# mindspore-lab/mindaudio

Hardware: AMD Instinct MI355X
Metric: utterances/s (16 kHz×10 s) fbanks+Conformer fwd, 1/2/4/8 MI355X (higher is better)
Workload: dtype bf16; 1 GPU; features.fbank (n_fft=512 hop=160 n_mels=80, batch-global top_db) on 64 x (10 s @16 kHz) synthetic waves per GPU -> Conformer-small encoder forward (12 blocks, d=256, 4 heads, ff=2048, conv k=15, eval mode) on the (64, 1000, 80) features; random-init weights; global_batch=64, frames=1000

## Files before the change

mindaudio_amd/csrc/subsample_fused.hip:

```cpp
#include <hip/hip_runtime.h>
#include <stdint.h>
#include <stdlib.h>

#include <type_traits>
#include <utility>

#include "../../include/mindaudio_amd.h"

#include "launch.h"

namespace ma {

typedef __attribute__((ext_vector_type(8))) __bf16 sf_bf16x8;
typedef __attribute__((ext_vector_type(4))) float sf_f32x4;
typedef __attribute__((ext_vector_type(2))) __bf16 sf_bf16x2;
typedef __attribute__((ext_vector_type(2))) float sf_f32x2;
typedef __attribute__((address_space(3))) void sf_lds_void_t;

template <int... Is, class F>
__device__ __forceinline__ void sf_static_for_impl(std::integer_sequence<int, Is...>, F&& f) {
  (f(std::integral_constant<int, Is>{}), ...);
}
template <int N, class F>
__device__ __forceinline__ void sf_static_for(F&& f) {
  sf_static_for_impl(std::make_integer_sequence<int, N>{}, f);
}

constexpr int kSfRows = 128, kSfC = 256, kSfThreads = 512;
constexpr int kSfIdim = 80, kSfF1 = 39, kSfF2 = 19;
constexpr int kSfNhoMax = 8;
constexpr int kSfH1Max = 2 * kSfNhoMax + 1;
constexpr int kSfInMax = 2 * kSfH1Max + 1;
constexpr int kSfPosMax = 672;
constexpr int kSfPitch = 80;
constexpr int kSfChunks = 8, kSfTaps = 9;
constexpr int kSfW2Bytes = kSfC * 9 * kSfC * 2;
constexpr int kSfOffX = 11264;
constexpr int kSfOffPatch = kSfOffX + kSfPosMax * 64;
constexpr int kSfPatchBytes = kSfPosMax * kSfPitch;
constexpr int kSfLds = kSfOffPatch + 2 * kSfPatchBytes;
constexpr int kSfOutPitch = 144;
static_assert(kSfInMax * kSfIdim <= 6 * kSfThreads && kSfPosMax <= 2 * kSfThreads && kSfLds <= 163840, "tile geometry");
static_assert(4 * kSfRows * kSfOutPitch <= kSfOffPatch + kSfPatchBytes, "epilogue staging must not reach patch buffer 1");

struct SubsampleFusedParams {
  const float* x;
  int64_t sb, st, sf;
  const float *mean, *istd;
  const char* packed;
  const float* b1;
  const float* b2;
  uint16_t* out;
  int32_t Ho, tiles_per_utt;
};

__device__ __forceinline__ uint32_t sf_pack_bf16(float lo, float hi) {
  const sf_bf16x2 r = __builtin_convertvector((sf_f32x2){lo, hi}, sf_bf16x2);
  return *reinterpret_cast<const uint32_t*>(&r);
}
__device__ __forceinline__ float sf_head(float x) { return __uint_as_float(sf_pack_bf16(x, 0.0f) << 16); }

template <bool IS_W>
__device__ __forceinline__ void sf_split_row(const float (&v)[9], uint32_t (&d)[16]) {
  float h[9], l[9];
#pragma unroll
  for (int t = 0; t < 9; ++t) {
    h[t] = sf_head(v[t]);
    l[t] = v[t] - h[t];
  }
  float k[32];
#pragma unroll
  for (int t = 0; t < 9; ++t) {
    k[t] = h[t];
    k[9 + t] = IS_W ? l[t] : h[t];
    k[18 + t] = IS_W ? h[t] : l[t];
  }
#pragma unroll
  for (int t = 27; t < 32; ++t) k[t] = 0.0f;
#pragma unroll
  for (int j = 0; j < 16; ++j) d[j] = sf_pack_bf16(k[2 * j], k[2 * j + 1]);
}

__global__ void subsample_fused_pack_kernel(const uint16_t* __restrict__ w2, const float* __restrict__ w1, uint4* __restrict__ out) {
  const int idx = blockIdx.x * blockDim.x + threadIdx.x;
  constexpr int kN2 = 4 * kSfChunks * kSfTaps * 4 * 64;
  if (idx < kN2) {
    const int lane = idx & 63, jt = (idx >> 6) & 3, ft = (idx >> 8) % (kSfChunks * kSfTaps), wv = (idx >> 8) / (kSfChunks * kSfTaps);
    const int cc = ft / kSfTaps, tap = ft - cc * kSfTaps;
    const int n = 64 * wv + 16 * jt + (lane & 15);
    out[idx] = *reinterpret_cast<const uint4*>(w2 + (int64_t)n * (9 * kSfC) + tap * kSfC + 32 * cc + 8 * (lane >> 4));
  } else if (idx < kN2 + 16 * 64) {
    const int j = idx - kN2, lane = j & 63, item = j >> 6;
    const int ch = 16 * item + (lane & 15), g = lane >> 4;
    float v[9];
#pragma unroll
    for (int t = 0; t < 9; ++t) v[t] = w1[ch * 9 + t];
    uint32_t d[16];
    sf_split_row<true>(v, d);
    out[idx] = g == 0 ? make_uint4(d[0], d[1], d[2], d[3]) : g == 1 ? make_uint4(d[4], d[5], d[6], d[7])
             : g == 2 ? make_uint4(d[8], d[9], d[10], d[11]) : make_uint4(d[12], d[13], d[14], d[15]);
  }
}

#ifndef SF_PRIO_C
#define SF_PRIO_C 1
#endif
#ifndef SF_PRIO_P
#define SF_PRIO_P 0
#endif
#ifdef MA_SF_PROF
__device__ unsigned long long g_sf_prof[2 * 3 * 32];
#define SF_STAMP(k) do { asm volatile("s_waitcnt lgkmcnt(0)" ::: "memory"); sf_ts[(k)] = __builtin_amdgcn_s_memtime(); asm volatile("s_waitcnt lgkmcnt(0)" ::: "memory"); } while (0)
#define SF_FLUSH(role)                                                                                        \
  do {                                                                                                        \
    const int slot_ = blockIdx.x == 0 ? 0 : blockIdx.x == 1200 ? 1 : blockIdx.x == 2300 ? 2 : -1;             \
    if (slot_ >= 0 && lane == 0)                                                                              \
      for (int k_ = 0; k_ < 32; ++k_) g_sf_prof[((role) * 3 + slot_) * 32 + k_] = sf_ts[k_];                  \
  } while (0)
#else
#define SF_STAMP(k) do { } while (0)
#define SF_FLUSH(role) do { } while (0)
#endif

__global__ __launch_bounds__(kSfThreads, 2) void subsample_fused_kernel(const SubsampleFusedParams p) {
  extern __shared__ __attribute__((aligned(16))) char smem[];
#ifdef MA_SF_PROF
  unsigned long long sf_ts[32] = {};
#endif
  SF_STAMP(0);
  const int tid = threadIdx.x, lane = tid & 63;
  const int wave = __builtin_amdgcn_readfirstlane(tid >> 6);
  const int b = blockIdx.x / p.tiles_per_utt, ti = blockIdx.x - b * p.tiles_per_utt;
  const int npos = p.Ho * kSfF2;
  const int p0 = ti * kSfRows;
  const int np = min(kSfRows, npos - p0);
  const int ho0 = p0 / kSfF2;
  const int nho = (p0 + np - 1) / kSfF2 - ho0 + 1;
  const int nh1 = 2 * nho + 1, nin = 2 * nh1 + 1;
  const int npatch = nh1 * kSfF1;
  float* rows = reinterpret_cast<float*>(smem);
  char* xim = smem + kSfOffX;
  char* patch = smem + kSfOffPatch;

  {
    const float* xb = p.x + (int64_t)b * p.sb + (int64_t)(4 * ho0) * p.st;
    const bool tfast = p.st <= p.sf;
    const int n = nin * kSfIdim;
    float v[6], mu[6], is[6];
    int dst[6];
#pragma unroll
    for (int j = 0; j < 6; ++j) {
      const int i = min(tid + kSfThreads * j, n - 1);
      const int r = tfast ? i % nin : i / kSfIdim, f = tfast ? i / nin : i % kSfIdim;
      dst[j] = r * kSfIdim + f;
      v[j] = xb[r * p.st + f * p.sf];
      mu[j] = p.mean ? p.mean[f] : 0.0f;
      is[j] = p.mean ? p.istd[f] : 1.0f;
    }
#pragma unroll
    for (int j = 0; j < 6; ++j)
      if (tid + kSfThreads * j < n) rows[dst[j]] = p.mean ? (v[j] - mu[j]) * is[j] : v[j];
  }
  __syncthreads();
  SF_STAMP(1);
#pragma unroll
  for (int j = 0; j < 2; ++j) {
    const int pos = tid + kSfThreads * j;
    if (pos < kSfPosMax) {
      uint32_t d[16];
      if (pos < npatch) {
        const int h = pos / kSfF1, w = pos - h * kSfF1;
        const float* in = rows + (2 * h) * kSfIdim + 2 * w;
        float v[9];
#pragma unroll
        for (int kh = 0; kh < 3; ++kh)
#pragma unroll
          for (int kw = 0; kw < 3; ++kw) v[kh * 3 + kw] = in[kh * kSfIdim + kw];
        sf_split_row<false>(v, d);
      } else {
#pragma unroll
        for (int q = 0; q < 16; ++q) d[q] = 0u;
      }
      uint4* xo = reinterpret_cast<uint4*>(xim + pos * 64);
      xo[0] = make_uint4(d[0], d[1], d[2], d[3]);
      xo[1] = make_uint4(d[4], d[5], d[6], d[7]);
      xo[2] = make_uint4(d[8], d[9], d[10], d[11]);
      xo[3] = make_uint4(d[12], d[13], d[14], d[15]);
    }
  }
  __syncthreads();
  SF_STAMP(2);

  const int ci = lane & 15, gi = lane >> 4;
  auto build_patch = [&](int cc, int pw, int nprod) __attribute__((always_inline)) {
    const uint4* w1f = reinterpret_cast<const uint4*>(p.packed + kSfW2Bytes) + (2 * cc) * 64 + lane;
    const uint4 wa = w1f[0], wb = w1f[64];
    const sf_bf16x8 a0 = *reinterpret_cast<const sf_bf16x8*>(&wa), a1 = *reinterpret_cast<const sf_bf16x8*>(&wb);
    const float4 ba = *reinterpret_cast<const float4*>(p.b1 + 32 * cc + 4 * gi);
    const float4 bb = *reinterpret_cast<const float4*>(p.b1 + 32 * cc + 16 + 4 * gi);
    const sf_f32x4 c0 = {ba.x, ba.y, ba.z, ba.w}, c1 = {bb.x, bb.y, bb.z, bb.w};
    const char* xsrc = xim + ci * 64 + gi * 16;
    char* dst = patch + (cc & 1) * kSfPatchBytes + ci * kSfPitch + gi * 8;
    const int ntile = (npatch + 15) >> 4;
    for (int pt = pw; pt < ntile; pt += nprod) {
      const uint4 xr = *reinterpret_cast<const uint4*>(xsrc + pt * (16 * 64));
      const sf_bf16x8 xf = *reinterpret_cast<const sf_bf16x8*>(&xr);
      const sf_f32x4 d0 = __builtin_amdgcn_mfma_f32_16x16x32_bf16(a0, xf, c0, 0, 0, 0);
      const sf_f32x4 d1 = __builtin_amdgcn_mfma_f32_16x16x32_bf16(a1, xf, c1, 0, 0, 0);
      char* o = dst + pt * (16 * kSfPitch);
      *reinterpret_cast<uint2*>(o) = make_uint2(sf_pack_bf16(fmaxf(d0[0], 0.f), fmaxf(d0[1], 0.f)), sf_pack_bf16(fmaxf(d0[2], 0.f), fmaxf(d0[3], 0.f)));
      *reinterpret_cast<uint2*>(o + 32) = make_uint2(sf_pack_bf16(fmaxf(d1[0], 0.f), fmaxf(d1[1], 0.f)), sf_pack_bf16(fmaxf(d1[2], 0.f), fmaxf(d1[3], 0.f)));
    }
  };
  build_patch(0, wave, 8);
  SF_STAMP(3);

  if (wave >= 4) {
#if SF_PRIO_P
    __builtin_amdgcn_s_setprio(SF_PRIO_P);
#endif
#pragma unroll 1
    for (int k = 0; k + 1 < kSfChunks; ++k) {
      __syncthreads();
      SF_STAMP(4 + 2 * k);
      build_patch(k + 1, wave - 4, 4);
      SF_STAMP(5 + 2 * k);
    }
    __syncthreads();
    SF_STAMP(20);
    if (wave == 4) SF_FLUSH(1);
    return;
  }

#if SF_PRIO_C
  __builtin_amdgcn_s_setprio(SF_PRIO_C);
#endif
  const int c = lane & 15, g = lane >> 4;
  uint32_t a_addr[8];
#pragma unroll
  for (int s = 0; s < 8; ++s) {
    int m = 16 * s + c;
    if (m >= np) m = np - 1;
    const int pos = p0 + m, ho = pos / kSfF2, wo = pos - ho * kSfF2;
    a_addr[s] = (uint32_t)(uintptr_t)(sf_lds_void_t*)(patch + ((2 * (ho - ho0)) * kSfF1 + 2 * wo) * kSfPitch + g * 16);
  }
  const uint32_t voff = lane * 16 + 2048;
  const char* wbase = p.packed + (int64_t)wave * (kSfChunks * kSfTaps) * 4096;
#define SF_LOAD(dst, ft, jt)                                                                                          \
  do {                                                                                                                \
    const char* cb_ = wbase + (int64_t)((ft) < kSfChunks * kSfTaps ? (ft) : kSfChunks * kSfTaps - 1) * 4096;          \
    asm volatile("global_load_dwordx4 %0, %1, %2 offset:%3" : "=v"(dst) : "v"(voff), "s"(cb_), "n"(((jt) - 2) * 1024) \
                 : "memory");                                                                                         \
  } while (0)
  sf_bf16x8 ring[8];
  sf_f32x4 acc[4][8];
  sf_bf16x8 af[2][8];
#define SF_LDS(dst, s_, imm_) asm volatile("ds_read_b128 %0, %1 offset:%2" : "=v"(dst) : "v"(a_addr[s_]), "n"(imm_) : "memory")
#define SF_LDS8(buf_, imm_)                                                                                   \
  SF_LDS(af[buf_][0], 0, imm_); SF_LDS(af[buf_][1], 1, imm_); SF_LDS(af[buf_][2], 2, imm_); SF_LDS(af[buf_][3], 3, imm_); \
  SF_LDS(af[buf_][4], 4, imm_); SF_LDS(af[buf_][5], 5, imm_); SF_LDS(af[buf_][6], 6, imm_); SF_LDS(af[buf_][7], 7, imm_)
  auto tap_step = [&](auto tapc, auto parc, auto bufc, int ft) __attribute__((always_inline)) {
    constexpr int TAP = decltype(tapc)::value, PAR = decltype(parc)::value, BUF = decltype(bufc)::value;
    constexpr int IMM = BUF * kSfPatchBytes + ((TAP / 3) * kSfF1 + (TAP % 3)) * kSfPitch;
    constexpr int NTAP = TAP + 1;
    constexpr int IMM_N = BUF * kSfPatchBytes + ((NTAP / 3) * kSfF1 + (NTAP % 3)) * kSfPitch;
    if constexpr (TAP == 0) { SF_LDS8(PAR, IMM); }
    if constexpr (TAP < kSfTaps - 1) {
      SF_LDS8(PAR ^ 1, IMM_N);
      asm volatile("s_waitcnt lgkmcnt(8)"
                   : "+v"(af[PAR][0]), "+v"(af[PAR][1]), "+v"(af[PAR][2]), "+v"(af[PAR][3]), "+v"(af[PAR][4]), "+v"(af[PAR][5]),
                     "+v"(af[PAR][6]), "+v"(af[PAR][7])::"memory");
    } else {
      asm volatile("s_waitcnt lgkmcnt(0)"
                   : "+v"(af[PAR][0]), "+v"(af[PAR][1]), "+v"(af[PAR][2]), "+v"(af[PAR][3]), "+v"(af[PAR][4]), "+v"(af[PAR][5]),
                     "+v"(af[PAR][6]), "+v"(af[PAR][7])::"memory");
    }
    sf_static_for<4>([&](auto tc) __attribute__((always_inline)) {
      constexpr int jt = decltype(tc)::value;
      constexpr int q = PAR * 4 + jt;
      asm volatile("s_waitcnt vmcnt(7)" : "+v"(ring[q])::"memory");
      sf_static_for<8>([&](auto sc) __attribute__((always_inline)) {
        constexpr int s = decltype(sc)::value;
        acc[jt][s] = __builtin_amdgcn_mfma_f32_16x16x32_bf16(ring[q], af[PAR][s], acc[jt][s], 0, 0, 0);
      });
      __builtin_amdgcn_sched_barrier(0);
      SF_LOAD(ring[q], ft + 2, jt);
    });
  };
  auto chunk_mfma = [&](auto bufc, int cc) __attribute__((always_inline)) {
    constexpr int BUF = decltype(bufc)::value;
    sf_static_for<kSfTaps>([&](auto tapc) __attribute__((always_inline)) {
      constexpr int TAP = decltype(tapc)::value;
      tap_step(tapc, std::integral_constant<int, (BUF + TAP) & 1>{}, bufc, cc * kSfTaps + TAP);
    });
  };

#pragma unroll
  for (int jt = 0; jt < 4; ++jt)
#pragma unroll
    for (int s = 0; s < 8; ++s) acc[jt][s] = sf_f32x4{0.f, 0.f, 0.f, 0.f};
  SF_LOAD(ring[0], 0, 0); SF_LOAD(ring[1], 0, 1); SF_LOAD(ring[2], 0, 2); SF_LOAD(ring[3], 0, 3);
  SF_LOAD(ring[4], 1, 0); SF_LOAD(ring[5], 1, 1); SF_LOAD(ring[6], 1, 2); SF_LOAD(ring[7], 1, 3);
  asm volatile("s_waitcnt lgkmcnt(0)" ::: "memory");
  __builtin_amdgcn_s_barrier();
#ifdef MA_SF_PROF
#pragma unroll
#else
#pragma unroll 1
#endif
  for (int cc = 0; cc < kSfChunks; cc += 2) {
    SF_STAMP(4 + 2 * cc);
    chunk_mfma(std::integral_constant<int, 0>{}, cc);
    SF_STAMP(5 + 2 * cc);
    __builtin_amdgcn_s_barrier();
    SF_STAMP(6 + 2 * cc);
    chunk_mfma(std::integral_constant<int, 1>{}, cc + 1);
    SF_STAMP(7 + 2 * cc);
    if (cc + 2 < kSfChunks) __builtin_amdgcn_s_barrier();
  }
  asm volatile("s_waitcnt vmcnt(0)"
               : "+v"(ring[0]), "+v"(ring[1]), "+v"(ring[2]), "+v"(ring[3]), "+v"(ring[4]), "+v"(ring[5]), "+v"(ring[6]), "+v"(ring[7])
               :
               : "memory");
#undef SF_LOAD
#undef SF_LDS
#undef SF_LDS8
  SF_STAMP(20);

  char* strip = smem + wave * (kSfRows * kSfOutPitch);
  float4 bv[4];
#pragma unroll
  for (int jt = 0; jt < 4; ++jt) bv[jt] = *reinterpret_cast<const float4*>(p.b2 + 64 * wave + 16 * jt + 4 * g);
#pragma unroll
  for (int s = 0; s < 8; ++s) {
    char* srow = strip + (16 * s + c) * kSfOutPitch + 8 * g;
#pragma unroll
    for (int jt = 0; jt < 4; ++jt) {
      const float v0 = fmaxf(acc[jt][s][0] + bv[jt].x, 0.f), v1 = fmaxf(acc[jt][s][1] + bv[jt].y, 0.f);
      const float v2 = fmaxf(acc[jt][s][2] + bv[jt].z, 0.f), v3 = fmaxf(acc[jt][s][3] + bv[jt].w, 0.f);
      *reinterpret_cast<uint2*>(srow + 32 * jt) = make_uint2(sf_pack_bf16(v0, v1), sf_pack_bf16(v2, v3));
    }
  }
  uint16_t* obase = p.out + ((int64_t)b * npos + p0) * kSfC + 64 * wave + 8 * (lane & 7);
#pragma unroll
  for (int it = 0; it < 16; ++it) {
    const int m = 8 * it + (lane >> 3);
    const uint4 v = *reinterpret_cast<const uint4*>(strip + m * kSfOutPitch + 16 * (lane & 7));
    if (m < np) *reinterpret_cast<uint4*>(obase + (int64_t)m * kSfC) = v;
  }
  SF_STAMP(21);
  if (wave == 0) SF_FLUSH(0);
}

#ifdef MA_SF_PROF
extern "C" int ma_debug_sf_prof(unsigned long long* host192) {
  return hipMemcpyFromSymbol(host192, HIP_SYMBOL(g_sf_prof), sizeof(unsigned long long) * 192) == hipSuccess ? 0 : -1;
}
#endif

MA_LDS_ATTR(subsample_fused_kernel, kSfLds);

}

using namespace ma;

extern "C" int64_t ma_subsample_fused_packed_bytes(int64_t idim, int64_t C) {
  if (idim != kSfIdim || C != kSfC) return MA_ERR_UNSUPPORTED;
  return (int64_t)kSfW2Bytes + 16 * 1024;
}

extern "C" int ma_subsample_fused_pack_bf16(const float* W1, const void* W2, int64_t idim, int64_t C, void* packed, ma_stream_t stream) {
  if (!W1 || !W2 || !packed) return MA_ERR_INVALID_ARG;
  if (ma_subsample_fused_packed_bytes(idim, C) < 0) return MA_ERR_UNSUPPORTED;
  if ((reinterpret_cast<uintptr_t>(W2) | reinterpret_cast<uintptr_t>(packed)) & 15) return MA_ERR_INVALID_ARG;
  const int total = 4 * kSfChunks * kSfTaps * 4 * 64 + 16 * 64;
  MA_LAUNCH(subsample_fused_pack_kernel, dim3((total + 255) / 256), dim3(256), 0, (hipStream_t)stream,
            reinterpret_cast<const uint16_t*>(W2), W1, reinterpret_cast<uint4*>(packed));
  return MA_OK;
}

extern "C" int ma_subsample_fused_bf16(const float* x, int64_t stride_b, int64_t stride_t, int64_t stride_f, int64_t batch, int64_t T,
                                       int32_t idim, const float* cmvn_mean, const float* cmvn_istd, const void* packed, const float* b1,
                                       const float* b2, int64_t C, void* out, ma_stream_t stream) {
  if (!x || !packed || !b1 || !b2 || !out || batch < 1 || T < 7) return MA_ERR_INVALID_ARG;
  if ((cmvn_mean == nullptr) != (cmvn_istd == nullptr)) return MA_ERR_INVALID_ARG;
  if (ma_subsample_fused_packed_bytes(idim, C) < 0) return MA_ERR_UNSUPPORTED;
  if ((reinterpret_cast<uintptr_t>(packed) | reinterpret_cast<uintptr_t>(out) | reinterpret_cast<uintptr_t>(b2) |
       reinterpret_cast<uintptr_t>(b1)) & 15)
    return MA_ERR_INVALID_ARG;
  const int64_t T1 = (T - 3) / 2 + 1, Ho = (T1 - 3) / 2 + 1;
  const int64_t tiles = (Ho * kSfF2 + kSfRows - 1) / kSfRows;
  if (batch * tiles > 0x7fffffff || Ho > (1 << 24)) return MA_ERR_UNSUPPORTED;
  SubsampleFusedParams p;
  p.x = x;
  p.sb = stride_b;
  p.st = stride_t;
  p.sf = stride_f;
  p.mean = cmvn_mean;
  p.istd = cmvn_istd;
  p.packed = reinterpret_cast<const char*>(packed);
  p.b1 = b1;
  p.b2 = b2;
  p.out = reinterpret_cast<uint16_t*>(out);
  p.Ho = (int32_t)Ho;
  p.tiles_per_utt = (int32_t)tiles;
  MA_LAUNCH(subsample_fused_kernel, dim3((unsigned)(batch * tiles)), dim3(kSfThreads), kSfLds, (hipStream_t)stream, p);
  return MA_OK;
}
```

Measured before the change: 33210 utterances/s.

## Make fused subsample conv kernel persistent with cross-tile prefetch overlap

After: 33510 utterances/s (median of 6 runs). Within noise of the previous version (+0.9%).

```diff
diff --git a/mindaudio_amd/csrc/subsample_fused.hip b/mindaudio_amd/csrc/subsample_fused.hip
--- a/mindaudio_amd/csrc/subsample_fused.hip
+++ b/mindaudio_amd/csrc/subsample_fused.hip
@@ -41,7 +41,8 @@
 constexpr int kSfLds = kSfOffPatch + 2 * kSfPatchBytes;
 constexpr int kSfOutPitch = 144;
 static_assert(kSfInMax * kSfIdim <= 6 * kSfThreads && kSfPosMax <= 2 * kSfThreads && kSfLds <= 163840, "tile geometry");
-static_assert(4 * kSfRows * kSfOutPitch <= kSfOffPatch + kSfPatchBytes, "epilogue staging must not reach patch buffer 1");
+static_assert(4 * kSfRows * kSfOutPitch <= kSfOffPatch + kSfPatchBytes, "tile form: epilogue staging must not reach patch buffer 1");
+static_assert(4 * (kSfRows / 2) * kSfOutPitch <= kSfPatchBytes, "persistent form: the half strips lie inside patch buffer 1");
 
 struct SubsampleFusedParams {
   const float* x;
@@ -52,6 +53,7 @@
   const float* b2;
   uint16_t* out;
   int32_t Ho, tiles_per_utt;
+  int32_t ntiles;
 };
 
 __device__ __forceinline__ uint32_t sf_pack_bf16(float lo, float hi) {
@@ -108,150 +110,194 @@
 #ifndef SF_PRIO_P
 #define SF_PRIO_P 0
 #endif
+#ifndef SF_PRE_TILES
+#define SF_PRE_TILES 12
+#endif
+static_assert(SF_PRE_TILES % 4 == 0, "whole rounds of the four producer waves");
 #ifdef MA_SF_PROF
 __device__ unsigned long long g_sf_prof[2 * 3 * 32];
+__device__ int g_sf_prof_tile;
 #define SF_STAMP(k) do { asm volatile("s_waitcnt lgkmcnt(0)" ::: "memory"); sf_ts[(k)] = __builtin_amdgcn_s_memtime(); asm volatile("s_waitcnt lgkmcnt(0)" ::: "memory"); } while (0)
+#define SF_STAMP_IF(c, k) do { if (c) SF_STAMP(k); } while (0)
+#define SF_FIRST (sf_which == 0)
+#define SF_T0 (sf_it == sf_which)
+#define SF_T1 (sf_it == sf_which + 1)
 #define SF_FLUSH(role)                                                                                        \
   do {                                                                                                        \
-    const int slot_ = blockIdx.x == 0 ? 0 : blockIdx.x == 1200 ? 1 : blockIdx.x == 2300 ? 2 : -1;             \
+    const int slot_ = blockIdx.x == 0 ? 0 : blockIdx.x == 100 ? 1 : blockIdx.x == 200 ? 2 : -1;               \
     if (slot_ >= 0 && lane == 0)                                                                              \
       for (int k_ = 0; k_ < 32; ++k_) g_sf_prof[((role) * 3 + slot_) * 32 + k_] = sf_ts[k_];                  \
   } while (0)
+#define SF_CHUNK_UNROLL _Pragma("unroll")
 #else
-#define SF_STAMP(k) do { } while (0)
+#define SF_STAMP_IF(c, k) do { } while (0)
 #define SF_FLUSH(role) do { } while (0)
-#endif
-
+#define SF_CHUNK_UNROLL _Pragma("unroll 1")
+#endif
+
+struct SfTile {
+  int b, p0, np, ho0, nin, npatch;
+};
+__device__ __forceinline__ SfTile sf_tile(const SubsampleFusedParams& p, int t) {
+  SfTile g;
+  g.b = t / p.tiles_per_utt;
+  const int ti = t - g.b * p.tiles_per_utt;
+  const int npos = p.Ho * kSfF2;
+  g.p0 = ti * kSfRows;
+  g.np = min(kSfRows, npos - g.p0);
+  g.ho0 = g.p0 / kSfF2;
+  const int nho = (g.p0 + g.np - 1) / kSfF2 - g.ho0 + 1;
+  const int nh1 = 2 * nho + 1;
+  g.nin = 2 * nh1 + 1;
+  g.npatch = nh1 * kSfF1;
+  return g;
+}
+
+template <int N>
+struct SfRowRegs {
+  float v[N], mu[N], is[N];
+  int dst[N];
+};
+template <int NTHR, bool CMVN_EARLY, int N>
+__device__ __forceinline__ void sf_rows_load(const SubsampleFusedParams& p, const SfTile& g, int id, SfRowRegs<N>& q) {
+  static_assert(kSfInMax * kSfIdim <= N * NTHR, "every element of the input rows has a thread");
+  const float* xb = p.x + (int64_t)g.b * p.sb + (int64_t)(4 * g.ho0) * p.st;
+  const bool tfast = p.st <= p.sf;
+  const int nin = g.nin, n = nin * kSfIdim, dv = tfast ? nin : kSfIdim;
+#pragma unroll
+  for (int j = 0; j < N; ++j) {
+    const int i = min(id + NTHR * j, n - 1);
+    const int qu = i / dv, re = i - qu * dv;
+    const int r = tfast ? re : qu, f = tfast ? qu : re;
+    q.dst[j] = r * kSfIdim + f;
+    q.v[j] = xb[r * p.st + f * p.sf];
+    if (CMVN_EARLY) {
+      q.mu[j] = p.mean ? p.mean[f] : 0.0f;
+      q.is[j] = p.mean ? p.istd[f] : 1.0f;
+    }
+  }
+}
+template <int NTHR, bool CMVN_EARLY, int N>
+__device__ __forceinline__ void sf_rows_store(const SubsampleFusedParams& p, const SfTile& g, int id, SfRowRegs<N>& q, float* rows) {
+  const int n = g.nin * kSfIdim;
+  if (!CMVN_EARLY) {
+#pragma unroll
+    for (int j = 0; j < N; ++j) {
+      const int f = q.dst[j] % kSfIdim;
+      q.mu[j] = p.mean ? p.mean[f] : 0.0f;
+      q.is[j] = p.mean ? p.istd[f] : 1.0f;
+    }
+  }
+#pragma unroll
+  for (int j = 0; j < N; ++j)
+    if (id + NTHR * j < n) rows[q.dst[j]] = p.mean ? (q.v[j] - q.mu[j]) * q.is[j] : q.v[j];
+}
+
+__device__ __forceinline__ void sf_build_x(const float* rows, char* xim, int pos, int npatch) {
+  uint32_t d[16];
+  if (pos < npatch) {
+    const int h = pos / kSfF1, w = pos - h * kSfF1;
+    const float* in = rows + (2 * h) * kSfIdim + 2 * w;
+    float v[9];
+#pragma unroll
+    for (int kh = 0; kh < 3; ++kh)
+#pragma unroll
+      for (int kw = 0; kw < 3; ++kw) v[kh * 3 + kw] = in[kh * kSfIdim + kw];
+    sf_split_row<false>(v, d);
+  } else {
+#pragma unroll
+    for (int q = 0; q < 16; ++q) d[q] = 0u;
+  }
+  uint4* xo = reinterpret_cast<uint4*>(xim + pos * 64);
+  xo[0] = make_uint4(d[0], d[1], d[2], d[3]);
+  xo[1] = make_uint4(d[4], d[5], d[6], d[7]);
+  xo[2] = make_uint4(d[8], d[9], d[10], d[11]);
+  xo[3] = make_uint4(d[12], d[13], d[14], d[15]);
+}
+
+struct SfPatchW {
+  sf_bf16x8 a0, a1;
+  sf_f32x4 c0, c1;
+};
+
+template <bool PERSIST>
 __global__ __launch_bounds__(kSfThreads, 2) void subsample_fused_kernel(const SubsampleFusedParams p) {
   extern __shared__ __attribute__((aligned(16))) char smem[];
 #ifdef MA_SF_PROF
   unsigned long long sf_ts[32] = {};
-#endif
-  SF_STAMP(0);
-  const int tid = threadIdx.x, lane = tid & 63;
+  const int sf_which = g_sf_prof_tile;
+  int sf_it = 0;
+#endif
+  SF_STAMP_IF(SF_FIRST, 0);
+  const int tid = threadIdx.x;
+  int lane = tid & 63;
   const int wave = __builtin_amdgcn_readfirstlane(tid >> 6);
-  const int b = blockIdx.x / p.tiles_per_utt, ti = blockIdx.x - b * p.tiles_per_utt;
   const int npos = p.Ho * kSfF2;
-  const int p0 = ti * kSfRows;
-  const int np = min(kSfRows, npos - p0);
-  const int ho0 = p0 / kSfF2;
-  const int nho = (p0 + np - 1) / kSfF2 - ho0 + 1;
-  const int nh1 = 2 * nho + 1, nin = 2 * nh1 + 1;
-  const int npatch = nh1 * kSfF1;
   float* rows = reinterpret_cast<float*>(smem);
   char* xim = smem + kSfOffX;
   char* patch = smem + kSfOffPatch;
+  int t = blockIdx.x;
+  SfTile g = sf_tile(p, t);
 
   {
-    const float* xb = p.x + (int64_t)b * p.sb + (int64_t)(4 * ho0) * p.st;
-    const bool tfast = p.st <= p.sf;
-    const int n = nin * kSfIdim;
-    float v[6], mu[6], is[6];
-    int dst[6];
-#pragma unroll
-    for (int j = 0; j < 6; ++j) {
-      const int i = min(tid + kSfThreads * j, n - 1);
-      const int r = tfast ? i % nin : i / kSfIdim, f = tfast ? i / nin : i % kSfIdim;
-      dst[j] = r * kSfIdim + f;
-      v[j] = xb[r * p.st + f * p.sf];
-      mu[j] = p.mean ? p.mean[f] : 0.0f;
-      is[j] = p.mean ? p.istd[f] : 1.0f;
-    }
-#pragma unroll
-    for (int j = 0; j < 6; ++j)
-      if (tid + kSfThreads * j < n) rows[dst[j]] = p.mean ? (v[j] - mu[j]) * is[j] : v[j];
+    SfRowRegs<6> q;
+    sf_rows_load<kSfThreads, true>(p, g, tid, q);
+    sf_rows_store<kSfThreads, true>(p, g, tid, q, rows);
   }
   __syncthreads();
-  SF_STAMP(1);
+  SF_STAMP_IF(SF_FIRST, 1);
 #pragma unroll
   for (int j = 0; j < 2; ++j) {
     const int pos = tid + kSfThreads * j;
-    if (pos < kSfPosMax) {
-      uint32_t d[16];
-      if (pos < npatch) {
-        const int h = pos / kSfF1, w = pos - h * kSfF1;
-        const float* in = rows + (2 * h) * kSfIdim + 2 * w;
-        float v[9];
-#pragma unroll
-        for (int kh = 0; kh < 3; ++kh)
-#pragma unroll
-          for (int kw = 0; kw < 3; ++kw) v[kh * 3 + kw] = in[kh * kSfIdim + kw];
-        sf_split_row<false>(v, d);
-      } else {
-#pragma unroll
-        for (int q = 0; q < 16; ++q) d[q] = 0u;
-      }
-      uint4* xo = reinterpret_cast<uint4*>(xim + pos * 64);
-      xo[0] = make_uint4(d[0], d[1], d[2], d[3]);
-      xo[1] = make_uint4(d[4], d[5], d[6], d[7]);
-      xo[2] = make_uint4(d[8], d[9], d[10], d[11]);
-      xo[3] = make_uint4(d[12], d[13], d[14], d[15]);
-    }
+    if (pos < kSfPosMax) sf_build_x(rows, xim, pos, g.npatch);
   }
   __syncthreads();
-  SF_STAMP(2);
-
-  const int ci = lane & 15, gi = lane >> 4;
-  auto build_patch = [&](int cc, int pw, int nprod) __attribute__((always_inline)) {
+  SF_STAMP_IF(SF_FIRST, 2);
+
+  int ci = lane & 15, gi = lane >> 4;
+  auto patch_w = [&](int cc) __attribute__((always_inline)) {
     const uint4* w1f = reinterpret_cast<const uint4*>(p.packed + kSfW2Bytes) + (2 * cc) * 64 + lane;
     const uint4 wa = w1f[0], wb = w1f[64];
-    const sf_bf16x8 a0 = *reinterpret_cast<const sf_bf16x8*>(&wa), a1 = *reinterpret_cast<const sf_bf16x8*>(&wb);
     const float4 ba = *reinterpret_cast<const float4*>(p.b1 + 32 * cc + 4 * gi);
     const float4 bb = *reinterpret_cast<const float4*>(p.b1 + 32 * cc + 16 + 4 * gi);
-    const sf_f32x4 c0 = {ba.x, ba.y, ba.z, ba.w}, c1 = {bb.x, bb.y, bb.z, bb.w};
+    SfPatchW w;
+    w.a0 = *reinterpret_cast<const sf_bf16x8*>(&wa);
+    w.a1 = *reinterpret_cast<const sf_bf16x8*>(&wb);
+    w.c0 = sf_f32x4{ba.x, ba.y, ba.z, ba.w};
+    w.c1 = sf_f32x4{bb.x, bb.y, bb.z, bb.w};
+    return w;
+  };
+  auto patch_run = [&](const SfPatchW& w, int cc, int pw, int nprod, int pt0, int pt1) __attribute__((always_inline)) {
     const char* xsrc = xim + ci * 64 + gi * 16;
     char* dst = patch + (cc & 1) * kSfPatchBytes + ci * kSfPitch + gi * 8;
-    const int ntile = (npatch + 15) >> 4;
-    for (int pt = pw; pt < ntile; pt += nprod) {
+    for (int pt = pt0 + pw; pt < pt1; pt += nprod) {
       const uint4 xr = *reinterpret_cast<const uint4*>(xsrc + pt * (16 * 64));
       const sf_bf16x8 xf = *reinterpret_cast<const sf_bf16x8*>(&xr);
-      const sf_f32x4 d0 = __builtin_amdgcn_mfma_f32_16x16x32_bf16(a0, xf, c0, 0, 0, 0);
-      const sf_f32x4 d1 = __builtin_amdgcn_mfma_f32_16x16x32_bf16(a1, xf, c1, 0, 0, 0);
+      const sf_f32x4 d0 = __builtin_amdgcn_mfma_f32_16x16x32_bf16(w.a0, xf, w.c0, 0, 0, 0);
+      const sf_f32x4 d1 = __builtin_amdgcn_mfma_f32_16x16x32_bf16(w.a1, xf, w.c1, 0, 0, 0);
       char* o = dst + pt * (16 * kSfPitch);
       *reinterpret_cast<uint2*>(o) = make_uint2(sf_pack_bf16(fmaxf(d0[0], 0.f), fmaxf(d0[1], 0.f)), sf_pack_bf16(fmaxf(d0[2], 0.f), fmaxf(d0[3], 0.f)));
       *reinterpret_cast<uint2*>(o + 32) = make_uint2(sf_pack_bf16(fmaxf(d1[0], 0.f), fmaxf(d1[1], 0.f)), sf_pack_bf16(fmaxf(d1[2], 0.f), fmaxf(d1[3], 0.f)));
     }
   };
-  build_patch(0, wave, 8);
-  SF_STAMP(3);
-
-  if (wave >= 4) {
-#if SF_PRIO_P
-    __builtin_amdgcn_s_setprio(SF_PRIO_P);
-#endif
-#pragma unroll 1
-    for (int k = 0; k + 1 < kSfChunks; ++k) {
-      __syncthreads();
-      SF_STAMP(4 + 2 * k);
-      build_patch(k + 1, wave - 4, 4);
-      SF_STAMP(5 + 2 * k);
-    }
-    __syncthreads();
-    SF_STAMP(20);
-    if (wave == 4) SF_FLUSH(1);
-    return;
-  }
-
-#if SF_PRIO_C
-  __builtin_amdgcn_s_setprio(SF_PRIO_C);
-#endif
-  const int c = lane & 15, g = lane >> 4;
-  uint32_t a_addr[8];
-#pragma unroll
-  for (int s = 0; s < 8; ++s) {
-    int m = 16 * s + c;
-    if (m >= np) m = np - 1;
-    const int pos = p0 + m, ho = pos / kSfF2, wo = pos - ho * kSfF2;
-    a_addr[s] = (uint32_t)(uintptr_t)(sf_lds_void_t*)(patch + ((2 * (ho - ho0)) * kSfF1 + 2 * wo) * kSfPitch + g * 16);
-  }
+  {
+    const SfPatchW w = patch_w(0);
+    patch_run(w, 0, wave, 8, 0, (g.npatch + 15) >> 4);
+  }
+  SF_STAMP_IF(SF_FIRST, 3);
+
   const uint32_t voff = lane * 16 + 2048;
-  const char* wbase = p.packed + (int64_t)wave * (kSfChunks * kSfTaps) * 4096;
+  const char* wbase = p.packed + (int64_t)(wave & 3) * (kSfChunks * kSfTaps) * 4096;
 #define SF_LOAD(dst, ft, jt)                                                                                          \
   do {                                                                                                                \
     const char* cb_ = wbase + (int64_t)((ft) < kSfChunks * kSfTaps ? (ft) : kSfChunks * kSfTaps - 1) * 4096;          \
     asm volatile("global_load_dwordx4 %0, %1, %2 offset:%3" : "=v"(dst) : "v"(voff), "s"(cb_), "n"(((jt) - 2) * 1024) \
                  : "memory");                                                                                         \
   } while (0)
+#define SF_LOAD_FIRST_TWO()                                                                          \
+  SF_LOAD(ring[0], 0, 0); SF_LOAD(ring[1], 0, 1); SF_LOAD(ring[2], 0, 2); SF_LOAD(ring[3], 0, 3);    \
+  SF_LOAD(ring[4], 1, 0); SF_LOAD(ring[5], 1, 1); SF_LOAD(ring[6], 1, 2); SF_LOAD(ring[7], 1, 3)
+  uint32_t a_addr[8];
   sf_bf16x8 ring[8];
   sf_f32x4 acc[4][8];
   sf_bf16x8 af[2][8];
@@ -294,61 +340,155 @@
       tap_step(tapc, std::integral_constant<int, (BUF + TAP) & 1>{}, bufc, cc * kSfTaps + TAP);
     });
   };
-
-#pragma unroll
-  for (int jt = 0; jt < 4; ++jt)
-#pragma unroll
-    for (int s = 0; s < 8; ++s) acc[jt][s] = sf_f32x4{0.f, 0.f, 0.f, 0.f};
-  SF_LOAD(ring[0], 0, 0); SF_LOAD(ring[1], 0, 1); SF_LOAD(ring[2], 0, 2); SF_LOAD(ring[3], 0, 3);
-  SF_LOAD(ring[4], 1, 0); SF_LOAD(ring[5], 1, 1); SF_LOAD(ring[6], 1, 2); SF_LOAD(ring[7], 1, 3);
-  asm volatile("s_waitcnt lgkmcnt(0)" ::: "memory");
-  __builtin_amdgcn_s_barrier();
+  auto epilogue = [&](char* strip, auto halvesc, const float4 (&bv)[4]) __attribute__((always_inline)) {
+    constexpr int HALVES = decltype(halvesc)::value, NS = 8 / HALVES, NIT = 16 / HALVES;
+    uint16_t* obase = p.out + ((int64_t)g.b * npos + g.p0) * kSfC + 64 * wave + 8 * (lane & 7);
+#pragma unroll
+    for (int h = 0; h < HALVES; ++h) {
+#pragma unroll
+      for (int s = h * NS; s < (h + 1) * NS; ++s) {
+        char* srow = strip + (16 * (s - h * NS) + ci) * kSfOutPitch + 8 * gi;
+#pragma unroll
+        for (int jt = 0; jt < 4; ++jt) {
+          const float v0 = fmaxf(acc[jt][s][0] + bv[jt].x, 0.f), v1 = fmaxf(acc[jt][s][1] + bv[jt].y, 0.f);
+          const float v2 = fmaxf(acc[jt][s][2] + bv[jt].z, 0.f), v3 = fmaxf(acc[jt][s][3] + bv[jt].w, 0.f);
+          *reinterpret_cast<uint2*>(srow + 32 * jt) = make_uint2(sf_pack_bf16(v0, v1), sf_pack_bf16(v2, v3));
+        }
+      }
+#pragma unroll
+      for (int it = h * NIT; it < (h + 1) * NIT; ++it) {
+        const int m = 8 * it + (lane >> 3);
+        const uint4 v = *reinterpret_cast<const uint4*>(strip + (m - h * (kSfRows / HALVES)) * kSfOutPitch + 16 * (lane & 7));
+        if (m < g.np) *reinterpret_cast<uint4*>(obase + (int64_t)m * kSfC) = v;
+      }
+    }
+  };
+
+  if (wave >= 4) {
+#if SF_PRIO_P
+    __builtin_amdgcn_s_setprio(SF_PRIO_P);
+#endif
+  } else {
+#if SF_PRIO_C
+    __builtin_amdgcn_s_setprio(SF_PRIO_C);
+#endif
+  }
+
+#pragma unroll 1
+  for (;;) {
+    const int64_t tn = (int64_t)t + gridDim.x;
+    const bool has_next = PERSIST && tn < p.ntiles;
+    SfTile gn = g;
+    if (has_next) gn = sf_tile(p, (int)tn);
+    int tidv = tid;
+    asm volatile("" : "+v"(tidv));
+    lane = tidv & 63;
+    ci = lane & 15;
+    gi = lane >> 4;
+    if (wave >= 4) {
+      const int pw = wave - 4, ptid = tidv - 4 * 64;
+      const int ntile = (g.npatch + 15) >> 4;
+      SF_STAMP_IF(SF_T0 && sf_it > 0, 0);
+      __syncthreads();
+      SF_STAMP_IF(SF_T0, 4);
+      {
+        const SfPatchW w = patch_w(1);
+        if (has_next) {
+          SfRowRegs<11> q;
+          sf_rows_load<kSfThreads / 2, false>(p, gn, ptid, q);
+          patch_run(w, 1, pw, 4, 0, ntile);
+          sf_rows_store<kSfThreads / 2, false>(p, gn, ptid, q, rows);
+        } else {
+          patch_run(w, 1, pw, 4, 0, ntile);
+        }
+      }
+      SF_STAMP_IF(SF_T0, 5);
+      SF_CHUNK_UNROLL
+      for (int k = 1; k + 1 < kSfChunks; ++k) {
+        __syncthreads();
+        SF_STAMP_IF(SF_T0, 4 + 2 * k);
+        const SfPatchW w = patch_w(k + 1);
+        patch_run(w, k + 1, pw, 4, 0, ntile);
+        SF_STAMP_IF(SF_T0, 5 + 2 * k);
+      }
+      __syncthreads();
+      SF_STAMP_IF(SF_T0, 20);
+      SfPatchW w0 = {};
+      const int ntile_n = has_next ? (gn.npatch + 15) >> 4 : 0;
+      if (has_next) {
+        w0 = patch_w(0);
+#pragma unroll
+        for (int j = 0; j < 3; ++j) {
+          const int tl = pw + 4 * (gi + 4 * j);
+          if (tl < kSfPosMax / 16) sf_build_x(rows, xim, 16 * tl + ci, gn.npatch);
+        }
+        asm volatile("" ::: "memory");
+        SF_STAMP_IF(SF_T0, 24);
+        patch_run(w0, 0, pw, 4, 0, min(ntile_n, SF_PRE_TILES));
+        SF_STAMP_IF(SF_T0, 25);
+      }
+      if constexpr (PERSIST) __syncthreads();
+      SF_STAMP_IF(SF_T0, 26);
+      if (has_next) patch_run(w0, 0, pw, 4, SF_PRE_TILES, ntile_n);
+      SF_STAMP_IF(SF_T0, 27);
+    } else {
+      SF_STAMP_IF(SF_T0 && sf_it > 0, 0);
+#pragma unroll
+      for (int jt = 0; jt < 4; ++jt)
+#pragma unroll
+        for (int s = 0; s < 8; ++s) acc[jt][s] = sf_f32x4{0.f, 0.f, 0.f, 0.f};
+      __builtin_amdgcn_s_waitcnt(0x0f70);
+      SF_LOAD_FIRST_TWO();
+#pragma unroll
+      for (int s = 0; s < 8; ++s) {
+        int m = 16 * s + ci;
+        if (m >= g.np) m = g.np - 1;
+        const int pos = g.p0 + m, ho = pos / kSfF2, wo = pos - ho * kSfF2;
+        a_addr[s] = (uint32_t)(uintptr_t)(sf_lds_void_t*)(patch + ((2 * (ho - g.ho0)) * kSfF1 + 2 * wo) * kSfPitch + gi * 16);
+      }
+      asm volatile("s_waitcnt lgkmcnt(0)" ::: "memory");
+      __builtin_amdgcn_s_barrier();
+      SF_CHUNK_UNROLL
+      for (int cc = 0; cc < kSfChunks; cc += 2) {
+        SF_STAMP_IF(SF_T0, 4 + 2 * cc);
+        SF_STAMP_IF(SF_T1 && cc == 0, 22);
+        chunk_mfma(std::integral_constant<int, 0>{}, cc);
+        SF_STAMP_IF(SF_T0, 5 + 2 * cc);
+        __builtin_amdgcn_s_barrier();
+        SF_STAMP_IF(SF_T0, 6 + 2 * cc);
+        chunk_mfma(std::integral_constant<int, 1>{}, cc + 1);
+        SF_STAMP_IF(SF_T0, 7 + 2 * cc);
+        if (cc + 2 < kSfChunks) __builtin_amdgcn_s_barrier();
+      }
+      float4 bv[4];
+#pragma unroll
+      for (int jt = 0; jt < 4; ++jt) bv[jt] = *reinterpret_cast<const float4*>(p.b2 + 64 * wave + 16 * jt + 4 * gi);
+      asm volatile("s_waitcnt vmcnt(0)"
+                   : "+v"(ring[0]), "+v"(ring[1]), "+v"(ring[2]), "+v"(ring[3]), "+v"(ring[4]), "+v"(ring[5]), "+v"(ring[6]), "+v"(ring[7])
+                   :
+                   : "memory");
+      SF_STAMP_IF(SF_T0, 20);
+      if constexpr (PERSIST) {
+        __builtin_amdgcn_s_barrier();
+        SF_STAMP_IF(SF_T0, 23);
+        epilogue(patch + kSfPatchBytes + wave * (kSfRows / 2 * kSfOutPitch), std::integral_constant<int, 2>{}, bv);
+      } else {
+        epilogue(smem + wave * (kSfRows * kSfOutPitch), std::integral_constant<int, 1>{}, bv);
+      }
+      SF_STAMP_IF(SF_T0, 21);
+    }
+    if (!has_next) break;
+    t = (int)tn;
+    g = gn;
 #ifdef MA_SF_PROF
-#pragma unroll
-#else
-#pragma unroll 1
-#endif
-  for (int cc = 0; cc < kSfChunks; cc += 2) {
-    SF_STAMP(4 + 2 * cc);
-    chunk_mfma(std::integral_constant<int, 0>{}, cc);
-    SF_STAMP(5 + 2 * cc);
-    __builtin_amdgcn_s_barrier();
-    SF_STAMP(6 + 2 * cc);
-    chunk_mfma(std::integral_constant<int, 1>{}, cc + 1);
-    SF_STAMP(7 + 2 * cc);
-    if (cc + 2 < kSfChunks) __builtin_amdgcn_s_barrier();
-  }
-  asm volatile("s_waitcnt vmcnt(0)"
-               : "+v"(ring[0]), "+v"(ring[1]), "+v"(ring[2]), "+v"(ring[3]), "+v"(ring[4]), "+v"(ring[5]), "+v"(ring[6]), "+v"(ring[7])
-               :
-               : "memory");
+    ++sf_it;
+#endif
+  }
 #undef SF_LOAD
+#undef SF_LOAD_FIRST_TWO
 #undef SF_LDS
 #undef SF_LDS8
-  SF_STAMP(20);
-
-  char* strip = smem + wave * (kSfRows * kSfOutPitch);
-  float4 bv[4];
-#pragma unroll
-  for (int jt = 0; jt < 4; ++jt) bv[jt] = *reinterpret_cast<const float4*>(p.b2 + 64 * wave + 16 * jt + 4 * g);
-#pragma unroll
-  for (int s = 0; s < 8; ++s) {
-    char* srow = strip + (16 * s + c) * kSfOutPitch + 8 * g;
-#pragma unroll
-    for (int jt = 0; jt < 4; ++jt) {
-      const float v0 = fmaxf(acc[jt][s][0] + bv[jt].x, 0.f), v1 = fmaxf(acc[jt][s][1] + bv[jt].y, 0.f);
-      const float v2 = fmaxf(acc[jt][s][2] + bv[jt].z, 0.f), v3 = fmaxf(acc[jt][s][3] + bv[jt].w, 0.f);
-      *reinterpret_cast<uint2*>(srow + 32 * jt) = make_uint2(sf_pack_bf16(v0, v1), sf_pack_bf16(v2, v3));
-    }
-  }
-  uint16_t* obase = p.out + ((int64_t)b * npos + p0) * kSfC + 64 * wave + 8 * (lane & 7);
-#pragma unroll
-  for (int it = 0; it < 16; ++it) {
-    const int m = 8 * it + (lane >> 3);
-    const uint4 v = *reinterpret_cast<const uint4*>(strip + m * kSfOutPitch + 16 * (lane & 7));
-    if (m < np) *reinterpret_cast<uint4*>(obase + (int64_t)m * kSfC) = v;
-  }
-  SF_STAMP(21);
+  if (wave == 4) SF_FLUSH(1);
   if (wave == 0) SF_FLUSH(0);
 }
 
@@ -356,9 +496,13 @@
 extern "C" int ma_debug_sf_prof(unsigned long long* host192) {
   return hipMemcpyFromSymbol(host192, HIP_SYMBOL(g_sf_prof), sizeof(unsigned long long) * 192) == hipSuccess ? 0 : -1;
 }
-#endif
-
-MA_LDS_ATTR(subsample_fused_kernel, kSfLds);
+extern "C" int ma_debug_sf_prof_tile(int tile) {
+  return hipMemcpyToSymbol(HIP_SYMBOL(g_sf_prof_tile), &tile, sizeof(int)) == hipSuccess ? 0 : -1;
+}
+#endif
+
+MA_LDS_ATTR(subsample_fused_kernel<true>, kSfLds);
+MA_LDS_ATTR(subsample_fused_kernel<false>, kSfLds);
 
 }
 
@@ -377,6 +521,26 @@
   MA_LAUNCH(subsample_fused_pack_kernel, dim3((total + 255) / 256), dim3(256), 0, (hipStream_t)stream,
             reinterpret_cast<const uint16_t*>(W2), W1, reinterpret_cast<uint4*>(packed));
   return MA_OK;
+}
+
+static bool sf_use_tile() {
+  static const bool use = [] {
+    const char* e = getenv("MINDAUDIO_AMD_SUBSAMPLE");
+    return e && e[0] == 't' && e[1] == 'i' && e[2] == 'l' && e[3] == 'e' && e[4] == 0;
+  }();
+  return use;
+}
+
+static int sf_num_cus() {
+  static int cached = 0;
+  if (!cached) {
+    int dev = 0;
+    hipDeviceProp_t prop;
+    if (hipGetDevice(&dev) == hipSuccess && hipGetDeviceProperties(&prop, dev) == hipSuccess && prop.multiProcessorCount > 0)
+      cached = prop.multiProcessorCount;
+    if (cached <= 0) cached = 256;
+  }
+  return cached;
 }
 
 extern "C" int ma_subsample_fused_bf16(const float* x, int64_t stride_b, int64_t stride_t, int64_t stride_f, int64_t batch, int64_t T,
@@ -404,6 +568,11 @@
   p.out = reinterpret_cast<uint16_t*>(out);
   p.Ho = (int32_t)Ho;
   p.tiles_per_utt = (int32_t)tiles;
-  MA_LAUNCH(subsample_fused_kernel, dim3((unsigned)(batch * tiles)), dim3(kSfThreads), kSfLds, (hipStream_t)stream, p);
+  p.ntiles = (int32_t)(batch * tiles);
+  if (sf_use_tile())
+    MA_LAUNCH(subsample_fused_kernel<false>, dim3((unsigned)p.ntiles), dim3(kSfThreads), kSfLds, (hipStream_t)stream, p);
+  else
+    MA_LAUNCH(subsample_fused_kernel<true>, dim3((unsigned)min(p.ntiles, sf_num_cus())), dim3(kSfThreads), kSfLds, (hipStream_t)stream,
+              p);
   return MA_OK;
 }
```
